# fabiocarrara/neural-ode-features

Measured on AMD Instinct MI355X. Metric: images/sec (fwd+adjoint) CIFAR-10 ODE-ResNet bs=128 at 1/2/4/8 GPU, higher is better.
Workload: dtype f32

## Files before the change

neural-ode-features_amd/csrc/kernels_stem.hip:

```cpp
#include "stem.h"
#include <type_traits>

namespace node {

namespace {

typedef float f32x16 __attribute__((ext_vector_type(16)));
typedef __bf16 bf16x8 __attribute__((ext_vector_type(8)));
typedef __bf16 bf16x2 __attribute__((ext_vector_type(2)));
typedef float f32x2 __attribute__((ext_vector_type(2)));
typedef unsigned u32x4 __attribute__((ext_vector_type(4)));

__device__ __forceinline__ void split3(float x, bf16_t& h, bf16_t& m, bf16_t& l) {
  const __bf16 bh = (__bf16)x;
  const float r = x - (float)bh;
  const __bf16 bm = (__bf16)r;
  const float r2 = r - (float)bm;
  const __bf16 bl = (__bf16)r2;
  h = __builtin_bit_cast(bf16_t, bh);
  m = __builtin_bit_cast(bf16_t, bm);
  l = __builtin_bit_cast(bf16_t, bl);
}
__device__ __forceinline__ void split8(const float4& p, const float4& q, u32x4& hh, u32x4& mm, u32x4& ll) {
  const f32x2 v[4] = {{p.x, p.y}, {p.z, p.w}, {q.x, q.y}, {q.z, q.w}};
// ... 322 lines not shown
    if (px >= a.OW) { px -= a.OW; py += 1; irow += cx_irow; }
    if (py >= a.OH) { py -= a.OH; irow += cy_irow; }
  };
  auto piece = [&](int ii, int stage) {
    const int inst = W + 4 * ii, im = inst / 6, part = (inst % 6) >> 1;
    const int kx = im >= 1 && im <= TG ? im - 1 : 0;
    const bf16_t* src = im == 0 ? dyb + part * a.dy_plane + dyo
                      : im > TG ? dy2b + part * a.dy_plane + dyo
                                : inb + part * a.in_plane + ino[kx];
    glds16(src, lds0 + stage * BUF + im * IMG + part * 2048 + H * 1024);
  };

  constexpr int NA = TG + (EX ? 1 : 0);
  f32x16 acc[NA];
#pragma unroll
  for (int j = 0; j < NA; ++j)
#pragma unroll
    for (int i = 0; i < 16; ++i) acc[j][i] = 0.f;

  constexpr int cob = W >> 1, cib = W & 1;
  const int kg = lane >> 5, g16 = (lane >> 4) & 1, m = lane & 15, tq = m >> 2, tp = m & 3;
  auto frag = [&](const unsigned char* img, int part, int cb0) -> bf16x8 {
    const int piece = ((cb0 + 16 * g16) >> 3) + (tp >> 1), inb8 = (tp & 1) << 3;
    const int r0 = 8 * kg + tq, r1 = r0 + 4;
    const s16x4 lo = __builtin_amdgcn_ds_read_tr16_b64_v4i16((__attribute__((address_space(3))) s16x4*)(img + part * 2048 + img_off<64>(r0, piece) + inb8));
    const s16x4 hi = __builtin_amdgcn_ds_read_tr16_b64_v4i16((__attribute__((address_space(3))) s16x4*)(img + part * 2048 + img_off<64>(r1, piece) + inb8));
    typedef short s16x8 __attribute__((ext_vector_type(8)));
    const s16x8 v = {lo[0], lo[1], lo[2], lo[3], hi[0], hi[1], hi[2], hi[3]};
    return __builtin_bit_cast(bf16x8, v);
  };

#pragma unroll
  for (int q = 0; q < D; ++q)
    if (q < nchunk) {
      sources();
#pragma unroll
      for (int ii = 0; ii < NP; ++ii) piece(ii, q);
    }
  int st_read = 0, st_fill = D;
  auto step = [&](int q, auto fill) {
    constexpr bool FILL = decltype(fill)::value;
    ring_step<NP, D>(q, nchunk);
    if constexpr (FILL) sources();
    const unsigned char* base = smem + st_read * BUF;
    bf16x8 fa[3], fb[TG][3], f2[3];
#pragma unroll
    for (int p = 0; p < 3; ++p) fa[p] = frag(base, p, 32 * cob);
#pragma unroll
    for (int j = 0; j < TG; ++j)
#pragma unroll
      for (int p = 0; p < 3; ++p) fb[j][p] = frag(base + (1 + j) * IMG, p, 32 * cib);
    if constexpr (EX) {
#pragma unroll
      for (int p = 0; p < 3; ++p) f2[p] = frag(base + (NIMG - 1) * IMG, p, 32 * cob);
    }
    int pk = 0;
    auto between = [&]() {
      if constexpr (FILL) {
        if (pk < NP) piece(pk, st_fill);
        ++pk;
        __builtin_amdgcn_sched_barrier(0);
      }
    };
    if constexpr (FILL) __builtin_amdgcn_sched_barrier(0);
#pragma unroll
    for (int j = 0; j < TG; ++j) {
      six_products(acc[j], fa, fb[j], between);
      if constexpr (EX) {
        if (j == 1) six_products(acc[TG], f2, fb[j], between);
      }
    }
    static_assert(NP <= 3 * NA, "a chunk's pieces go between its MFMA pairs");
    st_read = st_read + 1 == NST ? 0 : st_read + 1;
    st_fill = st_fill + 1 == NST ? 0 : st_fill + 1;
  };
  int q = 0;
  for (; q + D < nchunk; ++q) step(q, std::true_type());
  for (; q < nchunk; ++q) step(q, std::false_type());
  const int li = lane & 31, hh = lane >> 5;
  const int taps_total = TG * TG;
#pragma unroll
  for (int j = 0; j < NA; ++j) {
    float* dst = j < TG ? a.slab + ((size_t)split * taps_total + ky * TG + j) * a.Cout * a.Cin
                        : a.slab2 + (size_t)split * a.Cout * a.Cin;
#pragma unroll
    for (int i = 0; i < 16; ++i) {
      const int co = cot * 64 + 32 * cob + 8 * (i >> 2) + 4 * hh + (i & 3);
      dst[(size_t)co * a.Cin + cit * 64 + 32 * cib + li] = acc[j][i];
    }
  }
}

template <int TG, bool EX, int D>
__device__ __forceinline__ void stem_wgrad_waves(const SWgradArgs& a, unsigned char* smem, int wave) {
  if (wave == 0) stem_wgrad_wave<TG, EX, D, 0>(a, smem);
  else if (wave == 1) stem_wgrad_wave<TG, EX, D, 1>(a, smem);
  else if (wave == 2) stem_wgrad_wave<TG, EX, D, 2>(a, smem);
  else stem_wgrad_wave<TG, EX, D, 3>(a, smem);
}

template <int TG, bool EXTRA, int D>
__global__ __launch_bounds__(256) void k_stem_wgrad(const SWgradArgs a) {
  extern __shared__ __align__(16) unsigned char smem[];
  const int wave = __builtin_amdgcn_readfirstlane(threadIdx.x >> 6);
  if constexpr (EXTRA) {
    const int npair = (a.Cin >> 6) * (a.Cout >> 6);
    if ((blockIdx.x / npair) % 3 == 1) {
      stem_wgrad_waves<TG, true, D>(a, smem, wave);
      return;
    }
  }
  stem_wgrad_waves<TG, false, D>(a, smem, wave);
}

__global__ __launch_bounds__(256) void k_stem_conv0_fwd(const float* __restrict__ x, const float* __restrict__ w0t,
                                                        const float* __restrict__ bias, float* __restrict__ h0, int N, int Cin, int H,
                                                        int W) {
  const int t = threadIdx.x, lane = t & 63, wave = t >> 6, li = lane & 31, hh = lane >> 5;
  const int OH = H - 2, OW = W - 2, rows = N * OH * OW, K = 9 * Cin;
  const int row0 = (blockIdx.x * 4 + wave) * 32;
  if (row0 >= rows) return;
  const int r = row0 + li;
  const bool valid = r < rows;
  int base = 0;
  if (valid) {
    const int n = r / (OH * OW), rem = r - n * OH * OW, oy = rem / OW, ox = rem - oy * OW;
    base = (n * Cin * H + oy) * W + ox;
  }
  f32x16 acc0, acc1;
#pragma unroll
  for (int i = 0; i < 16; ++i) { acc0[i] = 0.f; acc1[i] = 0.f; }
  const int steps = (K + 1) >> 1;
  for (int s = 0; s < steps; ++s) {
    const int k = 2 * s + hh, kk = min(k, K - 1);
    const int ci = kk / 9, rem = kk - 9 * ci, ky = rem / 3, kx = rem - 3 * ky;
    const float av = valid ? x[base + (ci * H + ky) * W + kx] : 0.f;
    const float b0 = w0t[k * 64 + li], b1 = w0t[k * 64 + 32 + li];
    acc0 = __builtin_amdgcn_mfma_f32_32x32x2f32(av, b0, acc0, 0, 0, 0);
    acc1 = __builtin_amdgcn_mfma_f32_32x32x2f32(av, b1, acc1, 0, 0, 0);
  }
  const float bv0 = bias[li], bv1 = bias[32 + li];
#pragma unroll
  for (int i = 0; i < 16; ++i) {
    const int rr = row0 + 8 * (i >> 2) + 4 * hh + (i & 3);
    if (rr >= rows) continue;
    h0[(size_t)rr * 64 + li] = acc0[i] + bv0;
    h0[(size_t)rr * 64 + 32 + li] = acc1[i] + bv1;
  }
}

__global__ __launch_bounds__(256) void k_stem_conv0_wgrad(const float* __restrict__ x, const float* __restrict__ dh0,
                                                          float* __restrict__ slab, int N, int Cin, int H, int W, int rows_per_split) {
  __shared__ float red[2 * 16 * 64];
  const int t = threadIdx.x, lane = t & 63, wave = t >> 6, li = lane & 31, hh = lane >> 5;
  const int OH = H - 2, OW = W - 2, rows = N * OH * OW, K = 9 * Cin;
  const int per_wave = rows_per_split >> 2;
  const int rbeg = blockIdx.x * rows_per_split + wave * per_wave;
  const int rend = min(rbeg + per_wave, rows);
  int koff = 0;
  if (li < K) {
    const int ci = li / 9, rem = li - 9 * ci, ky = rem / 3;
    koff = (ci * H + ky) * W + (rem - 3 * ky);
  }
  int r = rbeg + hh;
  int n = 0, oy = 0, ox = 0;
  if (r < rows) {
    n = r / (OH * OW);
    const int rem = r - n * OH * OW;
    oy = rem / OW;
    ox = rem - oy * OW;
  }
  f32x16 acc0, acc1;
#pragma unroll
  for (int i = 0; i < 16; ++i) { acc0[i] = 0.f; acc1[i] = 0.f; }
  for (; r - hh < rend; r += 2) {
    const bool valid = r < rend;
    const float a0 = valid ? dh0[(size_t)r * 64 + li] : 0.f;
    const float a1 = valid ? dh0[(size_t)r * 64 + 32 + li] : 0.f;
    float bv = 0.f;
    if (valid) bv = li < K ? x[(n * Cin * H + oy) * W + ox + koff] : (li == K ? 1.f : 0.f);
    acc0 = __builtin_amdgcn_mfma_f32_32x32x2f32(a0, bv, acc0, 0, 0, 0);
    acc1 = __builtin_amdgcn_mfma_f32_32x32x2f32(a1, bv, acc1, 0, 0, 0);
    ox += 2;
    if (ox >= OW) {
      ox -= OW;
      oy += 1;
      if (oy >= OH) { oy = 0; n += 1; }
    }
  }
  for (int w = 1; w < 4; ++w) {
    if (wave == w) {
#pragma unroll
      for (int i = 0; i < 16; ++i) { red[i * 64 + lane] = acc0[i]; red[(16 + i) * 64 + lane] = acc1[i]; }
    }
    __syncthreads();
    if (wave == 0) {
#pragma unroll
      for (int i = 0; i < 16; ++i) { acc0[i] += red[i * 64 + lane]; acc1[i] += red[(16 + i) * 64 + lane]; }
    }
    __syncthreads();
  }
  if (wave != 0) return;
  float* dst = slab + (size_t)blockIdx.x * 64 * 32;
#pragma unroll
  for (int i = 0; i < 16; ++i) {
    const int co = 8 * (i >> 2) + 4 * hh + (i & 3);
    dst[co * 32 + li] = acc0[i];
    dst[(32 + co) * 32 + li] = acc1[i];
  }
}

constexpr int DG_TH = 8, DG_TW = 32, DG_PH = DG_TH + 2, DG_PW = DG_TW + 2, DG_NP = DG_PH * DG_PW, DG_NT = (DG_NP + 31) / 32, DG_PS = 29;
__global__ __launch_bounds__(256) void k_stem_conv0_dgrad(const float* __restrict__ dh0, const float* __restrict__ w0,
                                                          float* __restrict__ dx, int Cin, int H, int W, int tiles_x, int tiles_y) {
  __shared__ float P[DG_NT * 32 * DG_PS];
  const int t = threadIdx.x, lane = t & 63, wave = t >> 6, li = lane & 31, hh = lane >> 5;
  const int OH = H - 2, OW = W - 2, K = 9 * Cin;
  const int n = blockIdx.x / (tiles_x * tiles_y), rem = blockIdx.x - n * tiles_x * tiles_y, ty = rem / tiles_x, tx = rem - ty * tiles_x;
  const int y0 = ty * DG_TH, x0 = tx * DG_TW;
  float b[32];
#pragma unroll
  for (int s = 0; s < 32; ++s) b[s] = li < K ? w0[(32 * hh + s) * K + li] : 0.f;
  for (int tile = wave; tile < DG_NT; tile += 4) {
    const int pix = tile * 32 + li, py = pix / DG_PW, px = pix - py * DG_PW;
    const int oy = y0 - 2 + py, ox = x0 - 2 + px;
    const bool valid = pix < DG_NP && oy >= 0 && oy < OH && ox >= 0 && ox < OW;
    float4 av[8];
    if (valid) {
      const float4* src = reinterpret_cast<const float4*>(dh0 + ((size_t)(n * OH + oy) * OW + ox) * 64 + 32 * hh);
#pragma unroll
      for (int q = 0; q < 8; ++q) av[q] = src[q];
    } else {
#pragma unroll
      for (int q = 0; q < 8; ++q) av[q] = make_float4(0.f, 0.f, 0.f, 0.f);
    }
    f32x16 acc;
#pragma unroll
    for (int i = 0; i < 16; ++i) acc[i] = 0.f;
#pragma unroll
    for (int q = 0; q < 8; ++q) {
      acc = __builtin_amdgcn_mfma_f32_32x32x2f32(av[q].x, b[4 * q], acc, 0, 0, 0);
      acc = __builtin_amdgcn_mfma_f32_32x32x2f32(av[q].y, b[4 * q + 1], acc, 0, 0, 0);
      acc = __builtin_amdgcn_mfma_f32_32x32x2f32(av[q].z, b[4 * q + 2], acc, 0, 0, 0);
      acc = __builtin_amdgcn_mfma_f32_32x32x2f32(av[q].w, b[4 * q + 3], acc, 0, 0, 0);
    }
    if (li < 28) {
#pragma unroll
      for (int i = 0; i < 16; ++i) P[(tile * 32 + 8 * (i >> 2) + 4 * hh + (i & 3)) * DG_PS + li] = acc[i];
    }
  }
  __syncthreads();
  for (int idx = t; idx < Cin * DG_TH * DG_TW; idx += 256) {
    const int xx = idx % DG_TW, yy = (idx / DG_TW) % DG_TH, ci = idx / (DG_TW * DG_TH);
    const int y = y0 + yy, x = x0 + xx;
    if (y >= H || x >= W) continue;
    float s = 0.f;
#pragma unroll
    for (int ky = 0; ky < 3; ++ky)
#pragma unroll
      for (int kx = 0; kx < 3; ++kx) s += P[((yy + 2 - ky) * DG_PW + xx + 2 - kx) * DG_PS + ci * 9 + ky * 3 + kx];
    dx[((size_t)(n * Cin + ci) * H + y) * W + x] = s;
  }
}

__device__ __forceinline__ void group_sums(float v, float* red, float* grp, int CB, int cpg, int t) {
  red[t] = v;
  __syncthreads();
  const int ngrp = CB / cpg;
  if (t < ngrp) {
    float s = 0.f;
    for (int j = 0; j < 256 / CB; ++j)
      for (int k = 0; k < cpg; ++k) s += red[j * CB + t * cpg + k];
    grp[t] = s;
  }
  __syncthreads();
}

__global__ __launch_bounds__(256) void k_stem_gn_fwd(const SGnArgs a) {
  extern __shared__ __align__(16) unsigned char smem[];
  const int t = threadIdx.x;
  const int CB = a.CB, HW = a.HW, C = a.C;
  float* tile = reinterpret_cast<float*>(smem);
  float* red = tile + (size_t)HW * CB;
  float* gmean = red + 256;
  float* grstd = gmean + 128;
  const int nblk = C / CB;
  const int n = blockIdx.x / nblk, c0 = (blockIdx.x - n * nblk) * CB;
  const int q4 = CB >> 2;
  const float* src = a.h + ((size_t)n * HW) * C + c0;
  for (int idx = t; idx < HW * q4; idx += 256) {
    const int px = idx / q4, q = idx - px * q4;
    *reinterpret_cast<float4*>(tile + px * CB + 4 * q) = *reinterpret_cast<const float4*>(src + (size_t)px * C + 4 * q);
  }
  __syncthreads();
  const int c = t & (CB - 1), pg = t / CB, PG = 256 / CB;
  const float inv_m = 1.f / (float)(a.cpg * HW);
  float s = 0.f;
  for (int px = pg; px < HW; px += PG) s += tile[px * CB + c];
  group_sums(s, red, gmean, CB, a.cpg, t);
  const float mean = gmean[c / a.cpg] * inv_m;
  float s2 = 0.f;
  for (int px = pg; px < HW; px += PG) {
    const float d = tile[px * CB + c] - mean;
    s2 += d * d;
  }
  group_sums(s2, red, grstd, CB, a.cpg, t);
  const int ngrp = CB / a.cpg;
  if (t < ngrp) {
    const float m = gmean[t] * inv_m, rs = rsqrtf(grstd[t] * inv_m + a.eps);
    float* st = a.stats + ((size_t)n * (C / a.cpg) + c0 / a.cpg + t) * 2;
    st[0] = m;
    st[1] = rs;
  }
  __syncthreads();
  if (t < ngrp) {
    const float m = gmean[t] * inv_m, rs = rsqrtf(grstd[t] * inv_m + a.eps);
    gmean[t] = m;
    grstd[t] = rs;
  }
  __syncthreads();
  const int q8 = CB >> 3;
  for (int idx = t; idx < HW * q8; idx += 256) {
    const int px = idx / q8, q = idx - px * q8;
    const float4 p0 = *reinterpret_cast<const float4*>(tile + px * CB + 8 * q);
    const float4 p1 = *reinterpret_cast<const float4*>(tile + px * CB + 8 * q + 4);
    float v[8] = {p0.x, p0.y, p0.z, p0.w, p1.x, p1.y, p1.z, p1.w};
#pragma unroll
    for (int k = 0; k < 8; ++k) {
      const int cc = 8 * q + k, g = cc / a.cpg;
      const float y = (v[k] - gmean[g]) * grstd[g] * a.gamma[c0 + cc] + a.beta[c0 + cc];
      v[k] = fmaxf(y, 0.f);
    }
    u32x4 hh, mm, ll;
    split8(make_float4(v[0], v[1], v[2], v[3]), make_float4(v[4], v[5], v[6], v[7]), hh, mm, ll);
    bf16_t* dst = a.a3 + ((size_t)n * HW + px) * C + c0 + 8 * q;
    *reinterpret_cast<u32x4*>(dst) = hh;
    *reinterpret_cast<u32x4*>(dst + a.a_plane) = mm;
    *reinterpret_cast<u32x4*>(dst + 2 * a.a_plane) = ll;
  }
}

template <bool SKIP>
__global__ __launch_bounds__(256) void k_stem_gn_bwd(const SGnArgs a) {
  extern __shared__ __align__(16) unsigned char smem[];
  const int CB = a.CB, HW = a.HW, C = a.C;
  float* txh = reinterpret_cast<float*>(smem);
  float* tdy = txh + (size_t)HW * CB;
  float* redA = tdy + (size_t)HW * CB;
  float* redB = redA + 256;
  float* gmean = redB + 256;
  float* grstd = gmean + 128;
  float* gs1 = grstd + 128;
  float* gs2 = gs1 + 128;
  const int t = threadIdx.x;
  const int nblk = C / CB;
  const int n = blockIdx.x / nblk, c0 = (blockIdx.x - n * nblk) * CB;
  const int q4 = CB >> 2;
  const float* sh = a.h + ((size_t)n * HW) * C + c0;
  const float* sd = a.da + ((size_t)n * HW) * C + c0;
  for (int idx = t; idx < HW * q4; idx += 256) {
    const int px = idx / q4, q = idx - px * q4;
    *reinterpret_cast<float4*>(txh + px * CB + 4 * q) = *reinterpret_cast<const float4*>(sh + (size_t)px * C + 4 * q);
    *reinterpret_cast<float4*>(tdy + px * CB + 4 * q) = *reinterpret_cast<const float4*>(sd + (size_t)px * C + 4 * q);
  }
  const int ngrp = CB / a.cpg;
  if (t < ngrp) {
    const float* st = a.stats + ((size_t)n * (C / a.cpg) + c0 / a.cpg + t) * 2;
    gmean[t] = st[0];
    grstd[t] = st[1];
  }
  __syncthreads();
  const int c = t & (CB - 1), pg = t / CB, PG = 256 / CB;
  const float mean = gmean[c / a.cpg], rstd = grstd[c / a.cpg], gam = a.gamma[c0 + c], bet = a.beta[c0 + c];
  float sA = 0.f, sB = 0.f;
  for (int px = pg; px < HW; px += PG) {
    const float xh = (txh[px * CB + c] - mean) * rstd;
    const float y = xh * gam + bet;
    const float dy = y > 0.f ? tdy[px * CB + c] : 0.f;
    txh[px * CB + c] = xh;
    tdy[px * CB + c] = dy;
    sA += dy;
    sB += dy * xh;
  }
  redA[t] = sA;
  redB[t] = sB;
  __syncthreads();
  if (t < CB) {
    float A = 0.f, B = 0.f;
    for (int j = 0; j < PG; ++j) { A += redA[j * CB + t]; B += redB[j * CB + t]; }
    a.gpart[((size_t)n * 2 + 0) * C + c0 + t] = B;
    a.gpart[((size_t)n * 2 + 1) * C + c0 + t] = A;
    redA[t] = A * gam;
    redB[t] = B * gam;
  }
  __syncthreads();
  if (t < ngrp) {
    float s1 = 0.f, s2 = 0.f;
    for (int k = 0; k < a.cpg; ++k) { s1 += redA[t * a.cpg + k]; s2 += redB[t * a.cpg + k]; }
    gs1[t] = s1;
    gs2[t] = s2;
  }
  __syncthreads();
  const float inv_m = 1.f / (float)(a.cpg * HW);
  const int q8 = CB >> 3;
  for (int idx = t; idx < HW * q8; idx += 256) {
    const int px = idx / q8, q = idx - px * q8;
    float v[8];
#pragma unroll
    for (int k = 0; k < 8; ++k) {
      const int cc = 8 * q + k, g = cc / a.cpg;
      const float xh = txh[px * CB + cc], dy = tdy[px * CB + cc];
      v[k] = grstd[g] * (dy * a.gamma[c0 + cc] - (gs1[g] + xh * gs2[g]) * inv_m);
    }
    const size_t o = ((size_t)n * HW + px) * C + c0 + 8 * q;
    if constexpr (SKIP) {
      const float4 k0 = *reinterpret_cast<const float4*>(a.skip + o), k1 = *reinterpret_cast<const float4*>(a.skip + o + 4);
      v[0] += k0.x; v[1] += k0.y; v[2] += k0.z; v[3] += k0.w;
      v[4] += k1.x; v[5] += k1.y; v[6] += k1.z; v[7] += k1.w;
    }
    const float4 p0 = make_float4(v[0], v[1], v[2], v[3]), p1 = make_float4(v[4], v[5], v[6], v[7]);
    if (a.dh) {
      *reinterpret_cast<float4*>(a.dh + o) = p0;
      *reinterpret_cast<float4*>(a.dh + o + 4) = p1;
    }
    if (a.dh3) {
      u32x4 hh, mm, ll;
      split8(p0, p1, hh, mm, ll);
      *reinterpret_cast<u32x4*>(a.dh3 + o) = hh;
      *reinterpret_cast<u32x4*>(a.dh3 + o + a.dh_plane) = mm;
      *reinterpret_cast<u32x4*>(a.dh3 + o + 2 * a.dh_plane) = ll;
    }
  }
}

__global__ __launch_bounds__(256) void k_stem_from_nchw(const float* __restrict__ src, float* __restrict__ dst, bf16_t* __restrict__ dst3,
                                                        size_t plane, int C, int HW, float* __restrict__ bpart) {
  __shared__ float tile[64][65];
  const int t = threadIdx.x;
  const int npb = (HW + 63) / 64, ncb = C / 64;
  const int n = blockIdx.x / (npb * ncb), rem = blockIdx.x - n * npb * ncb, cb = rem / npb, pb = rem - cb * npb;
  const int c0 = cb * 64, p0 = pb * 64;
  for (int idx = t; idx < 64 * 64; idx += 256) {
    const int cc = idx >> 6, pp = idx & 63;
    tile[cc][pp] = p0 + pp < HW ? src[((size_t)n * C + c0 + cc) * HW + p0 + pp] : 0.f;
  }
  __syncthreads();
  if (bpart != nullptr && t < 64) {
    float s = 0.f;
#pragma unroll 8
    for (int pp = 0; pp < 64; ++pp) s += tile[t][pp];
    bpart[((size_t)n * npb + pb) * C + c0 + t] = s;
  }
  for (int idx = t; idx < 64 * 8; idx += 256) {
    const int pp = idx >> 3, q = idx & 7;
    if (p0 + pp >= HW) continue;
    float v[8];
#pragma unroll
    for (int k = 0; k < 8; ++k) v[k] = tile[8 * q + k][pp];
    const size_t o = ((size_t)n * HW + p0 + pp) * C + c0 + 8 * q;
    const float4 a0 = make_float4(v[0], v[1], v[2], v[3]), a1 = make_float4(v[4], v[5], v[6], v[7]);
    if (dst) {
      *reinterpret_cast<float4*>(dst + o) = a0;
      *reinterpret_cast<float4*>(dst + o + 4) = a1;
    }
    if (dst3) {
      u32x4 hh, mm, ll;
      split8(a0, a1, hh, mm, ll);
      *reinterpret_cast<u32x4*>(dst3 + o) = hh;
      *reinterpret_cast<u32x4*>(dst3 + o + plane) = mm;
      *reinterpret_cast<u32x4*>(dst3 + o + 2 * plane) = ll;
    }
  }
}

__global__ __launch_bounds__(256) void k_stem_colsum(const float* __restrict__ src, float* __restrict__ part, int rows, int C, int rows_per_blk) {
  __shared__ float red[4][64];
  const int t = threadIdx.x, cl = t & 63, sub = t >> 6;
  const int nct = C >> 6;
  const int blk = blockIdx.x / nct, c = (blockIdx.x - blk * nct) * 64 + cl;
  const int r0 = blk * rows_per_blk, r1 = min(r0 + rows_per_blk, rows);
  float s0 = 0.f, s1 = 0.f;
  int r = r0 + sub;
  for (; r + 4 < r1; r += 8) {
    s0 += src[(size_t)r * C + c];
    s1 += src[(size_t)(r + 4) * C + c];
  }
  if (r < r1) s0 += src[(size_t)r * C + c];
  red[sub][cl] = s0 + s1;
  __syncthreads();
  if (sub == 0) part[(size_t)blk * C + c] = (red[0][cl] + red[1][cl]) + (red[2][cl] + red[3][cl]);
}

__global__ __launch_bounds__(256) void k_stem_split(const float* __restrict__ src, bf16_t* __restrict__ dst3, size_t plane, size_t n8) {
  const size_t i = (size_t)blockIdx.x * 256 + threadIdx.x;
  if (i >= n8) return;
  const float4 a0 = reinterpret_cast<const float4*>(src)[2 * i], a1 = reinterpret_cast<const float4*>(src)[2 * i + 1];
  u32x4 hh, mm, ll;
  split8(a0, a1, hh, mm, ll);
  *reinterpret_cast<u32x4*>(dst3 + 8 * i) = hh;
  *reinterpret_cast<u32x4*>(dst3 + 8 * i + plane) = mm;
  *reinterpret_cast<u32x4*>(dst3 + 8 * i + 2 * plane) = ll;
}

__global__ __launch_bounds__(256) void k_stem_to_nchw(const float* __restrict__ src, float* __restrict__ dst, int C, int HW) {
  __shared__ float tile[64][65];
  const int t = threadIdx.x;
  const int npb = (HW + 63) / 64, ncb = C / 64;
  const int n = blockIdx.x / (npb * ncb), rem = blockIdx.x - n * npb * ncb, cb = rem / npb, pb = rem - cb * npb;
  const int c0 = cb * 64, p0 = pb * 64;
  for (int idx = t; idx < 64 * 64; idx += 256) {
    const int pp = idx >> 6, cc = idx & 63;
    tile[cc][pp] = p0 + pp < HW ? src[((size_t)n * HW + p0 + pp) * C + c0 + cc] : 0.f;
  }
  __syncthreads();
  for (int idx = t; idx < 64 * 64; idx += 256) {
    const int cc = idx >> 6, pp = idx & 63;
    if (p0 + pp < HW) dst[((size_t)n * C + c0 + cc) * HW + p0 + pp] = tile[cc][pp];
  }
}

__global__ __launch_bounds__(256) void k_stem_prep(const SPrepArgs a) {
  int seg = 0;
  while (seg < 7 && blockIdx.x >= a.blk0[seg + 1]) ++seg;
  const size_t idx = (size_t)(blockIdx.x - a.blk0[seg]) * 256 + threadIdx.x;
  const int job = seg < 6 ? seg : a.njobs + (seg - 6);
  if (job < a.njobs) {
    const SPrepJob& j = a.job[job];
    const size_t total = (size_t)j.taps * j.Cout * j.Cin;
    if (idx >= total) return;
    const int ci = (int)(idx % j.Cin);
    const size_t r = idx / j.Cin;
    const int co = (int)(r % j.Cout), tap = (int)(r / j.Cout);
    const float v = j.w[((size_t)co * j.Cin + ci) * j.taps + tap];
    bf16_t h, m, l;
    split3(v, h, m, l);
    const size_t of = ((size_t)tap * j.Cout + co) * j.Cin + ci, od = ((size_t)tap * j.Cin + ci) * j.Cout + co;
    j.wf[of] = h; j.wf[of + total] = m; j.wf[of + 2 * total] = l;
    j.wd[od] = h; j.wd[od + total] = m; j.wd[od + 2 * total] = l;
    return;
  }
  if (job == a.njobs) {
    if (a.w0t == nullptr || idx >= 28 * 64) return;
    const int k = (int)(idx / 64), co = (int)(idx % 64);
    a.w0t[idx] = k < a.k0 ? a.w0[co * a.k0 + k] : 0.f;
    return;
  }
  const int which = (int)(idx / 4096), e = (int)(idx % 4096);
  if (which >= a.nzero * 3) return;
  const int ten = which / 3, p = which - 3 * ten;
  if (e < a.zero_c[ten]) a.zero[ten][p * a.zero_plane[ten] + e] = 0;
}

__global__ __launch_bounds__(256) void k_stem_reduce(const SReduceArgs a) {
  __shared__ float part[4][64];
  int ji = 0;
  while (ji + 1 < a.njobs && blockIdx.x >= a.blk0[ji + 1]) ++ji;
  const SReduceJob& j = a.job[ji];
  const unsigned bx = blockIdx.x - a.blk0[ji];
  const int t = threadIdx.x;
  if (j.kind == 0) {
    const int co = bx / j.taps, tap = bx - co * j.taps;
    if (co >= j.Co) return;
    const size_t total = (size_t)j.taps * j.Co * j.Ci;
    const int cl = t & 63, sub = t >> 6;
    for (int c0 = 0; c0 < j.Ci; c0 += 64) {
      const float* src = j.slab + ((size_t)tap * j.Co + co) * j.Ci + c0 + cl;
      float s0 = 0.f, s1 = 0.f;
      int k = sub;
      for (; k + 28 < j.ns; k += 32) {
        float v[8];
#pragma unroll
        for (int q = 0; q < 8; ++q) v[q] = src[(size_t)(k + 4 * q) * total];
#pragma unroll
        for (int q = 0; q < 8; q += 2) { s0 += v[q]; s1 += v[q + 1]; }
      }
      for (; k + 4 < j.ns; k += 8) {
        s0 += src[(size_t)k * total];
        s1 += src[(size_t)(k + 4) * total];
      }
      if (k < j.ns) s0 += src[(size_t)k * total];
      part[sub][cl] = s0 + s1;
      __syncthreads();
      if (sub == 0) j.out[((size_t)co * j.Ci + c0 + cl) * j.taps + tap] = (part[0][cl] + part[1][cl]) + (part[2][cl] + part[3][cl]);
      __syncthreads();
    }
  } else {
    const size_t nout = j.kind == 1 ? (size_t)64 * 32 : j.kind == 2 ? (size_t)2 * j.Co : (size_t)j.Co;
    const int o = t & 31, g = t >> 5;
    const size_t idx = (size_t)bx * 32 + o;
    if ((size_t)bx * 32 >= nout) return;
    const bool on = idx < nout;
    const float* src = j.slab + (on ? idx : 0);
    float acc = 0.f;
    int k = g;
    for (; k + 56 < j.ns; k += 64) {
      float v[8];
#pragma unroll
      for (int q = 0; q < 8; ++q) v[q] = src[(size_t)(k + 8 * q) * nout];
      acc += ((v[0] + v[1]) + (v[2] + v[3])) + ((v[4] + v[5]) + (v[6] + v[7]));
    }
    for (; k < j.ns; k += 8) acc += src[(size_t)k * nout];
    part[g >> 1][(g & 1) * 32 + o] = acc;
    __syncthreads();
    if (g != 0 || !on) return;
    const float sum = ((part[0][o] + part[0][32 + o]) + (part[1][o] + part[1][32 + o])) + ((part[2][o] + part[2][32 + o]) + (part[3][o] + part[3][32 + o]));
    if (j.kind == 1) {
      const int co = (int)(idx >> 5), kk = (int)(idx & 31);
      if (kk < j.Ci) j.out[co * j.Ci + kk] = sum;
      else if (kk == j.Ci) j.out2[co] = sum;
    } else {
      if (idx < (size_t)j.Co) j.out[idx] = sum;
      else j.out2[idx - j.Co] = sum;
    }
  }
}

}

static bool stem_ring() { return env_int("NODE_TUNE_STEM_RING", 1) != 0; }

void launch_stem_conv(const SConvArgs& a, hipStream_t s) {
  const int mt = a.cls_tile0[a.nclass];
  const int ntn = (a.Cout / 64) * ((a.mode == 0 && a.w2 != nullptr) ? 2 : 1);
#define STEM_CONV(KC, D)                                                                  \
  {                                                                                       \
    static bool attr[MAX_DEVICES] = {};                                                   \
    allow_full_lds(reinterpret_cast<const void*>(k_stem_conv<KC, D>), attr);              \
    const size_t lds = (size_t)(D + 1) * (3 * 128 + 3 * 64) * 2 * KC + 512;               \
    hipLaunchKernelGGL((k_stem_conv<KC, D>), dim3(mt * ntn), dim3(256), lds, s, a);        \
  }
  if (stem_ring()) STEM_CONV(32, STEM_RING_D)
  else STEM_CONV(64, 1)
#undef STEM_CONV
}

void launch_stem_wgrad(const SWgradArgs& a, hipStream_t s) {
  const int taps = a.KH * a.KW;
  const int krows = stem_wgrad_rows(taps);
  const int grid = (a.Cin / 64) * (a.Cout / 64) * krows * a.nsplit;
  const int nimg = 1 + krows + (a.dy23 ? 1 : 0);
#define STEM_WG(T, EX, D)                                                                \
  {                                                                                       \
    static bool attr[MAX_DEVICES] = {};                                                   \
    allow_full_lds(reinterpret_cast<const void*>(k_stem_wgrad<T, EX, D>), attr);          \
    const size_t lds = (size_t)(D + 1) * nimg * 3 * 16 * 128;                             \
    hipLaunchKernelGGL((k_stem_wgrad<T, EX, D>), dim3(grid), dim3(256), lds, s, a);        \
  }
  if (stem_ring()) {
    if (taps == 9 && a.dy23) STEM_WG(3, true, STEM_RING_D)
    else if (taps == 9) STEM_WG(3, false, STEM_RING_D)
    else if (taps == 16) STEM_WG(4, false, STEM_RING_D)
    else STEM_WG(1, false, STEM_RING_D)
  } else {
    if (taps == 9 && a.dy23) STEM_WG(3, true, 1)
    else if (taps == 9) STEM_WG(3, false, 1)
    else if (taps == 16) STEM_WG(4, false, 1)
    else STEM_WG(1, false, 1)
  }
#undef STEM_WG
}

void launch_stem_conv0_fwd(const float* x, const float* w0t, const float* bias, float* h0, int N, int Cin, int H, int W, hipStream_t s) {
  const int rows = N * (H - 2) * (W - 2);
  hipLaunchKernelGGL(k_stem_conv0_fwd, dim3((rows + 127) / 128), dim3(256), 0, s, x, w0t, bias, h0, N, Cin, H, W);
}
void launch_stem_conv0_wgrad(const float* x, const float* dh0, float* slab, int N, int Cin, int H, int W, int nsplit, int rows_per_split,
                             hipStream_t s) {
  hipLaunchKernelGGL(k_stem_conv0_wgrad, dim3(nsplit), dim3(256), 0, s, x, dh0, slab, N, Cin, H, W, rows_per_split);
}
void launch_stem_conv0_dgrad(const float* dh0, const float* w0, float* dx, int N, int Cin, int H, int W, hipStream_t s) {
  const int tx = (W + DG_TW - 1) / DG_TW, ty = (H + DG_TH - 1) / DG_TH;
  hipLaunchKernelGGL(k_stem_conv0_dgrad, dim3((unsigned)(N * tx * ty)), dim3(256), 0, s, dh0, w0, dx, Cin, H, W, tx, ty);
}

int stem_gn_cb(int HW, int C, int cpg) {
  const size_t budget = 150 * 1024;
  int cb = 8;
  while (cb < cpg) cb *= 2;
  if (cb > C || cb > 128 || (size_t)HW * cb * 2 * sizeof(float) > budget) return 0;
  while (cb * 2 <= C && cb * 2 <= 128 && (size_t)HW * cb * 4 * sizeof(float) <= budget) cb *= 2;
  static const int cap = env_int("NODE_TUNE_STEM_GNCB", -1);
  while (cap > 0 && cb > cap && cb / 2 >= cpg && cb / 2 >= 8) cb /= 2;
  if (C % cb != 0 || cb % cpg != 0) return 0;
  return cb;
}
void launch_stem_gn_fwd(const SGnArgs& a, hipStream_t s) {
  static bool attr[MAX_DEVICES] = {};
  allow_full_lds(reinterpret_cast<const void*>(k_stem_gn_fwd), attr);
  hipLaunchKernelGGL(k_stem_gn_fwd, dim3(a.N * (a.C / a.CB)), dim3(256), ((size_t)a.HW * a.CB + 512) * sizeof(float), s, a);
}
void launch_stem_gn_bwd(const SGnArgs& a, hipStream_t s) {
  const dim3 grid(a.N * (a.C / a.CB));
  const size_t lds = ((size_t)2 * a.HW * a.CB + 1024) * sizeof(float);
  if (a.skip) {
    static bool attr[MAX_DEVICES] = {};
    allow_full_lds(reinterpret_cast<const void*>(k_stem_gn_bwd<true>), attr);
    hipLaunchKernelGGL(k_stem_gn_bwd<true>, grid, dim3(256), lds, s, a);
  } else {
    static bool attr[MAX_DEVICES] = {};
    allow_full_lds(reinterpret_cast<const void*>(k_stem_gn_bwd<false>), attr);
    hipLaunchKernelGGL(k_stem_gn_bwd<false>, grid, dim3(256), lds, s, a);
  }
}

void launch_stem_prep(const SPrepArgs& a0, hipStream_t s) {
  SPrepArgs a = a0;
  unsigned at = 0;
  for (int i = 0; i < 6; ++i) {
    a.blk0[i] = at;
    if (i < a.njobs) at += (unsigned)(((size_t)a.job[i].taps * a.job[i].Cout * a.job[i].Cin + 255) / 256);
  }
  a.blk0[6] = at; at += (28 * 64 + 255) / 256;
  a.blk0[7] = at; at += (unsigned)(((size_t)a.nzero * 3 * 4096 + 255) / 256);
  a.blk0[8] = at;
  hipLaunchKernelGGL(k_stem_prep, dim3(at), dim3(256), 0, s, a);
}
void launch_stem_from_nchw(const float* src, float* dst_nhwc, bf16_t* dst3, size_t plane, int N, int C, int HW, hipStream_t s, float* bpart) {
  hipLaunchKernelGGL(k_stem_from_nchw, dim3(N * (C / 64) * ((HW + 63) / 64)), dim3(256), 0, s, src, dst_nhwc, dst3, plane, C, HW, bpart);
}
void launch_stem_colsum(const float* src, float* part, int rows, int C, int rows_per_blk, hipStream_t s) {
  const int nblk = (rows + rows_per_blk - 1) / rows_per_blk;
  hipLaunchKernelGGL(k_stem_colsum, dim3(nblk * (C / 64)), dim3(256), 0, s, src, part, rows, C, rows_per_blk);
}
void launch_stem_split(const float* src, bf16_t* dst3, size_t plane, size_t n, hipStream_t s) {
  hipLaunchKernelGGL(k_stem_split, dim3((unsigned)((n / 8 + 255) / 256)), dim3(256), 0, s, src, dst3, plane, n / 8);
}
void launch_stem_to_nchw(const float* src_nhwc, float* dst, int N, int C, int HW, hipStream_t s) {
  hipLaunchKernelGGL(k_stem_to_nchw, dim3(N * (C / 64) * ((HW + 63) / 64)), dim3(256), 0, s, src_nhwc, dst, C, HW);
}
void launch_stem_reduce(const SReduceArgs& a0, hipStream_t s) {
  SReduceArgs a = a0;
  unsigned at = 0;
  for (int i = 0; i < a.njobs; ++i) {
    const SReduceJob& j = a.job[i];
    a.blk0[i] = at;
    at += (unsigned)(j.kind == 0 ? j.Co * j.taps : j.kind == 1 ? 64 : j.kind == 2 ? (2 * j.Co + 31) / 32 : (j.Co + 31) / 32);
  }
  a.blk0[a.njobs] = at;
  if (at == 0) return;
  hipLaunchKernelGGL(k_stem_reduce, dim3(at), dim3(256), 0, s, a);
}

}
```

Before: 30300.

## Add batched-load GroupNorm stem kernels with XCD-aware block remapping

Adds new forward and backward GroupNorm kernels for the stem, enabled by default. Each thread issues eight float4 global loads before writing any of them to LDS, which raises memory-level parallelism during the tile fill. Division and modulo are replaced with shifts based on log2 sizes. Block IDs are remapped round-robin across 8 chunks, apparently to group neighbouring blocks on one XCD, and the group reductions are unrolled. The risk is higher register pressure from the batched loads, and the shift arithmetic assumes power-of-two CB and cpg.

```diff
diff --git a/neural-ode-features_amd/csrc/kernels_stem.hip b/neural-ode-features_amd/csrc/kernels_stem.hip
--- a/neural-ode-features_amd/csrc/kernels_stem.hip
+++ b/neural-ode-features_amd/csrc/kernels_stem.hip
@@ -648,7 +648,7 @@
   float s2 = 0.f;
   for (int px = pg; px < HW; px += PG) {
     const float d = tile[px * CB + c] - mean;
-    s2 += d * d;
+    s2 = __builtin_fmaf(d, d, s2);
   }
   group_sums(s2, red, grstd, CB, a.cpg, t);
   const int ngrp = CB / a.cpg;
@@ -779,6 +779,259 @@
   }
 }
 
+constexpr int GN_NB = 8;
+__device__ __forceinline__ int gn_log2(int v) { return 31 - __clz(v); }
+__device__ __forceinline__ int gn_block_id() {
+  const int b = blockIdx.x, q = gridDim.x >> 3, r = gridDim.x & 7, x = b & 7;
+  return (x < r ? x * (q + 1) : r * (q + 1) + (x - r) * q) + (b >> 3);
+}
+
+template <int NS>
+__device__ __forceinline__ void gn_fill(float* tile0, const float* __restrict__ src0, float* tile1, const float* __restrict__ src1,
+                                        float* dump, int C, int lq4, int total, int t) {
+  const int qm = (1 << lq4) - 1;
+  int idx = t;
+  for (; idx + (GN_NB - 1) * 256 < total; idx += GN_NB * 256) {
+    float4 r0[GN_NB], r1[GN_NB];
+#pragma unroll
+    for (int u = 0; u < GN_NB; ++u) {
+      const int i = idx + 256 * u;
+      const size_t o = (size_t)(i >> lq4) * C + 4 * (i & qm);
+      r0[u] = *reinterpret_cast<const float4*>(src0 + o);
+      if constexpr (NS == 2) r1[u] = *reinterpret_cast<const float4*>(src1 + o);
+    }
+#pragma unroll
+    for (int u = 0; u < GN_NB; ++u) {
+      *reinterpret_cast<float4*>(tile0 + 4 * (idx + 256 * u)) = r0[u];
+      if constexpr (NS == 2) *reinterpret_cast<float4*>(tile1 + 4 * (idx + 256 * u)) = r1[u];
+    }
+  }
+  if (idx < total) {
+    float4 r0[GN_NB], r1[GN_NB];
+#pragma unroll
+    for (int u = 0; u < GN_NB; ++u) {
+      const int i = min(idx + 256 * u, total - 1);
+      const size_t o = (size_t)(i >> lq4) * C + 4 * (i & qm);
+      r0[u] = *reinterpret_cast<const float4*>(src0 + o);
+      if constexpr (NS == 2) r1[u] = *reinterpret_cast<const float4*>(src1 + o);
+    }
+#pragma unroll
+    for (int u = 0; u < GN_NB; ++u) {
+      const bool real = idx + 256 * u < total;
+      *reinterpret_cast<float4*>(real ? tile0 + 4 * (idx + 256 * u) : dump) = r0[u];
+      if constexpr (NS == 2) *reinterpret_cast<float4*>(real ? tile1 + 4 * (idx + 256 * u) : dump) = r1[u];
+    }
+  }
+}
+
+__device__ __forceinline__ void group_sums_ahead(float v, float* red, float* grp, int CB, int lcpg, int PG, int t) {
+  red[t] = v;
+  __syncthreads();
+  if (t < (CB >> lcpg)) {
+    const float* r0 = red + (t << lcpg);
+    const int n = PG << lcpg, km = (1 << lcpg) - 1;
+    float s = 0.f;
+    for (int i = 0; i < n; i += 8) {
+      float x[8];
+#pragma unroll
+      for (int u = 0; u < 8; ++u) {
+        const int ii = min(i + u, n - 1);
+        x[u] = r0[(ii >> lcpg) * CB + (ii & km)];
+      }
+#pragma unroll
+      for (int u = 0; u < 8; ++u)
+        if (i + u < n) s += x[u];
+    }
+    grp[t] = s;
+  }
+  __syncthreads();
+}
+
+__global__ __launch_bounds__(256) void k_stem_gn_fwd_fl(const SGnArgs a) {
+  extern __shared__ __align__(16) unsigned char smem[];
+  const int t = threadIdx.x;
+  const int CB = a.CB, HW = a.HW, C = a.C;
+  float* tile = reinterpret_cast<float*>(smem);
+  float* red = tile + (size_t)HW * CB;
+  float* gmean = red + 256;
+  float* grstd = gmean + 128;
+  const int nblk = C / CB, bid = gn_block_id();
+  const int n = bid / nblk, c0 = (bid - n * nblk) * CB;
+  const int lcb = gn_log2(CB), lcpg = gn_log2(a.cpg);
+  gn_fill<1>(tile, a.h + ((size_t)n * HW) * C + c0, nullptr, nullptr, red, C, lcb - 2, HW << (lcb - 2), t);
+  __syncthreads();
+  const int c = t & (CB - 1), pg = t >> lcb, PG = 256 >> lcb;
+  const float inv_m = 1.f / (float)(a.cpg * HW);
+  float s = 0.f;
+#pragma unroll 4
+  for (int px = pg; px < HW; px += PG) s += tile[px * CB + c];
+  group_sums_ahead(s, red, gmean, CB, lcpg, PG, t);
+  const float mean = gmean[c >> lcpg] * inv_m;
+  float s2 = 0.f;
+#pragma unroll 4
+  for (int px = pg; px < HW; px += PG) {
+    const float d = tile[px * CB + c] - mean;
+    s2 = __builtin_fmaf(d, d, s2);
+  }
+  group_sums_ahead(s2, red, grstd, CB, lcpg, PG, t);
+  const int ngrp = CB >> lcpg;
+  if (t < ngrp) {
+    const float m = gmean[t] * inv_m, rs = rsqrtf(grstd[t] * inv_m + a.eps);
+    float* st = a.stats + ((size_t)n * (C >> lcpg) + (c0 >> lcpg) + t) * 2;
+    st[0] = m;
+    st[1] = rs;
+  }
+  __syncthreads();
+  if (t < ngrp) {
+    const float m = gmean[t] * inv_m, rs = rsqrtf(grstd[t] * inv_m + a.eps);
+    gmean[t] = m;
+    grstd[t] = rs;
+  }
+  __syncthreads();
+  const int lq8 = lcb - 3, q = t & ((1 << lq8) - 1), pstep = 256 >> lq8;
+  float gm[8], gr[8], ga[8], be[8];
+#pragma unroll
+  for (int k = 0; k < 8; ++k) {
+    const int cc = 8 * q + k, g = cc >> lcpg;
+    gm[k] = gmean[g];
+    gr[k] = grstd[g];
+    ga[k] = a.gamma[c0 + cc];
+    be[k] = a.beta[c0 + cc];
+  }
+#pragma unroll 2
+  for (int px = t >> lq8; px < HW; px += pstep) {
+    const float4 p0 = *reinterpret_cast<const float4*>(tile + px * CB + 8 * q);
+    const float4 p1 = *reinterpret_cast<const float4*>(tile + px * CB + 8 * q + 4);
+    float v[8] = {p0.x, p0.y, p0.z, p0.w, p1.x, p1.y, p1.z, p1.w};
+#pragma unroll
+    for (int k = 0; k < 8; ++k) {
+      const float y = (v[k] - gm[k]) * gr[k] * ga[k] + be[k];
+      v[k] = fmaxf(y, 0.f);
+    }
+    u32x4 hh, mm, ll;
+    split8(make_float4(v[0], v[1], v[2], v[3]), make_float4(v[4], v[5], v[6], v[7]), hh, mm, ll);
+    bf16_t* dst = a.a3 + ((size_t)n * HW + px) * C + c0 + 8 * q;
+    *reinterpret_cast<u32x4*>(dst) = hh;
+    *reinterpret_cast<u32x4*>(dst + a.a_plane) = mm;
+    *reinterpret_cast<u32x4*>(dst + 2 * a.a_plane) = ll;
+  }
+}
+
+template <bool SKIP>
+__global__ __launch_bounds__(256) void k_stem_gn_bwd_fl(const SGnArgs a) {
+  extern __shared__ __align__(16) unsigned char smem[];
+  const int CB = a.CB, HW = a.HW, C = a.C;
+  float* txh = reinterpret_cast<float*>(smem);
+  float* tdy = txh + (size_t)HW * CB;
+  float* redA = tdy + (size_t)HW * CB;
+  float* redB = redA + 256;
+  float* gmean = redB + 256;
+  float* grstd = gmean + 128;
+  float* gs1 = grstd + 128;
+  float* gs2 = gs1 + 128;
+  const int t = threadIdx.x;
+  const int nblk = C / CB, bid = gn_block_id();
+  const int n = bid / nblk, c0 = (bid - n * nblk) * CB;
+  const int lcb = gn_log2(CB), lcpg = gn_log2(a.cpg);
+  gn_fill<2>(txh, a.h + ((size_t)n * HW) * C + c0, tdy, a.da + ((size_t)n * HW) * C + c0, redA, C, lcb - 2, HW << (lcb - 2), t);
+  const int ngrp = CB >> lcpg;
+  if (t < ngrp) {
+    const float* st = a.stats + ((size_t)n * (C >> lcpg) + (c0 >> lcpg) + t) * 2;
+    gmean[t] = st[0];
+    grstd[t] = st[1];
+  }
+  __syncthreads();
+  const int c = t & (CB - 1), pg = t >> lcb, PG = 256 >> lcb;
+  const float mean = gmean[c >> lcpg], rstd = grstd[c >> lcpg], gam = a.gamma[c0 + c], bet = a.beta[c0 + c];
+  float sA = 0.f, sB = 0.f;
+#pragma unroll 4
+  for (int px = pg; px < HW; px += PG) {
+    const float xh = (txh[px * CB + c] - mean) * rstd;
+    const float y = xh * gam + bet;
+    const float dy = y > 0.f ? tdy[px * CB + c] : 0.f;
+    txh[px * CB + c] = xh;
+    tdy[px * CB + c] = dy;
+    sA += dy;
+    sB += dy * xh;
+  }
+  redA[t] = sA;
+  redB[t] = sB;
+  __syncthreads();
+  if (t < CB) {
+    float A = 0.f, B = 0.f;
+    for (int j0 = 0; j0 < PG; j0 += 8) {
+      float xa[8], xb[8];
+#pragma unroll
+      for (int u = 0; u < 8; ++u) {
+        const int j = min(j0 + u, PG - 1);
+        xa[u] = redA[j * CB + t];
+        xb[u] = redB[j * CB + t];
+      }
+#pragma unroll
+      for (int u = 0; u < 8; ++u)
+        if (j0 + u < PG) { A += xa[u]; B += xb[u]; }
+    }
+    a.gpart[((size_t)n * 2 + 0) * C + c0 + t] = B;
+    a.gpart[((size_t)n * 2 + 1) * C + c0 + t] = A;
+    redA[t] = A * gam;
+    redB[t] = B * gam;
+  }
+  __syncthreads();
+  if (t < ngrp) {
+    float s1 = 0.f, s2 = 0.f;
+    for (int k = 0; k < a.cpg; ++k) { s1 += redA[t * a.cpg + k]; s2 += redB[t * a.cpg + k]; }
+    gs1[t] = s1;
+    gs2[t] = s2;
+  }
+  __syncthreads();
+  const float inv_m = 1.f / (float)(a.cpg * HW);
+  const int lq8 = lcb - 3, q = t & ((1 << lq8) - 1), pstep = 256 >> lq8;
+  float gr[8], ga[8], g1[8], g2[8];
+#pragma unroll
+  for (int k = 0; k < 8; ++k) {
+    const int cc = 8 * q + k, g = cc >> lcpg;
+    gr[k] = grstd[g];
+    ga[k] = a.gamma[c0 + cc];
+    g1[k] = gs1[g];
+    g2[k] = gs2[g];
+  }
+  constexpr int PX_PER_TRIP = SKIP ? 1 : 2;
+#pragma unroll PX_PER_TRIP
+  for (int px = t >> lq8; px < HW; px += pstep) {
+    const size_t o = ((size_t)n * HW + px) * C + c0 + 8 * q;
+    float4 k0, k1;
+    if constexpr (SKIP) {
+      k0 = *reinterpret_cast<const float4*>(a.skip + o);
+      k1 = *reinterpret_cast<const float4*>(a.skip + o + 4);
+    }
+    const float4 x0 = *reinterpret_cast<const float4*>(txh + px * CB + 8 * q), x1 = *reinterpret_cast<const float4*>(txh + px * CB + 8 * q + 4);
+    const float4 d0 = *reinterpret_cast<const float4*>(tdy + px * CB + 8 * q), d1 = *reinterpret_cast<const float4*>(tdy + px * CB + 8 * q + 4);
+    const float xs[8] = {x0.x, x0.y, x0.z, x0.w, x1.x, x1.y, x1.z, x1.w}, ds[8] = {d0.x, d0.y, d0.z, d0.w, d1.x, d1.y, d1.z, d1.w};
+    float v[8];
+#pragma unroll
+    for (int k = 0; k < 8; ++k) {
+      const float xh = xs[k], dy = ds[k];
+      v[k] = gr[k] * (dy * ga[k] - (g1[k] + xh * g2[k]) * inv_m);
+    }
+    if constexpr (SKIP) {
+      v[0] += k0.x; v[1] += k0.y; v[2] += k0.z; v[3] += k0.w;
+      v[4] += k1.x; v[5] += k1.y; v[6] += k1.z; v[7] += k1.w;
+    }
+    const float4 p0 = make_float4(v[0], v[1], v[2], v[3]), p1 = make_float4(v[4], v[5], v[6], v[7]);
+    if (a.dh) {
+      *reinterpret_cast<float4*>(a.dh + o) = p0;
+      *reinterpret_cast<float4*>(a.dh + o + 4) = p1;
+    }
+    if (a.dh3) {
+      u32x4 hh, mm, ll;
+      split8(p0, p1, hh, mm, ll);
+      *reinterpret_cast<u32x4*>(a.dh3 + o) = hh;
+      *reinterpret_cast<u32x4*>(a.dh3 + o + a.dh_plane) = mm;
+      *reinterpret_cast<u32x4*>(a.dh3 + o + 2 * a.dh_plane) = ll;
+    }
+  }
+}
+
 __global__ __launch_bounds__(256) void k_stem_from_nchw(const float* __restrict__ src, float* __restrict__ dst, bf16_t* __restrict__ dst3,
                                                         size_t plane, int C, int HW, float* __restrict__ bpart) {
   __shared__ float tile[64][65];
@@ -1030,7 +1283,14 @@
   if (C % cb != 0 || cb % cpg != 0) return 0;
   return cb;
 }
+static bool stem_gn_fl() { return env_int("NODE_TUNE_STEM_GN", 1) != 0; }
 void launch_stem_gn_fwd(const SGnArgs& a, hipStream_t s) {
+  if (stem_gn_fl()) {
+    static bool attr[MAX_DEVICES] = {};
+    allow_full_lds(reinterpret_cast<const void*>(k_stem_gn_fwd_fl), attr);
+    hipLaunchKernelGGL(k_stem_gn_fwd_fl, dim3(a.N * (a.C / a.CB)), dim3(256), ((size_t)a.HW * a.CB + 512) * sizeof(float), s, a);
+    return;
+  }
   static bool attr[MAX_DEVICES] = {};
   allow_full_lds(reinterpret_cast<const void*>(k_stem_gn_fwd), attr);
   hipLaunchKernelGGL(k_stem_gn_fwd, dim3(a.N * (a.C / a.CB)), dim3(256), ((size_t)a.HW * a.CB + 512) * sizeof(float), s, a);
@@ -1038,6 +1298,18 @@
 void launch_stem_gn_bwd(const SGnArgs& a, hipStream_t s) {
   const dim3 grid(a.N * (a.C / a.CB));
   const size_t lds = ((size_t)2 * a.HW * a.CB + 1024) * sizeof(float);
+  if (stem_gn_fl()) {
+    if (a.skip) {
+      static bool attr[MAX_DEVICES] = {};
+      allow_full_lds(reinterpret_cast<const void*>(k_stem_gn_bwd_fl<true>), attr);
+      hipLaunchKernelGGL(k_stem_gn_bwd_fl<true>, grid, dim3(256), lds, s, a);
+    } else {
+      static bool attr[MAX_DEVICES] = {};
+      allow_full_lds(reinterpret_cast<const void*>(k_stem_gn_bwd_fl<false>), attr);
+      hipLaunchKernelGGL(k_stem_gn_bwd_fl<false>, grid, dim3(256), lds, s, a);
+    }
+    return;
+  }
   if (a.skip) {
     static bool attr[MAX_DEVICES] = {};
     allow_full_lds(reinterpret_cast<const void*>(k_stem_gn_bwd<true>), attr);
```

After: 30750, median of 6. 1.02x the previous value.
